# jw007123/hp-Adaptive-Signed-Distance-Field-Octree

Measured on AMD Instinct MI355X. Metric: Query() Mpts/sec at targetError=1e-5 (union3 field, 10M SplitMix64 pts per GPU, HBM-resident); Create() ms reported as create_ms, higher is better.
Workload: dtype f64

## Files before the change

hp-adaptive-signed-distance-field-octree_amd/__init__.py:

```python
import ctypes as C
import os

import numpy as np

_HERE = os.path.dirname(os.path.abspath(__file__))
_WHICH = os.environ.get("HPSDF_LIBRARY", "")
LIB_PATH = os.path.join(_HERE, "lib", "libhpsdf_%s.so" % _WHICH if _WHICH else "libhpsdf.so")
_LIB = None

OK = 0
ERR_INVALID_ARGUMENT = 1
ERR_NO_DEVICE = 2
ERR_HIP = 3
ERR_BAD_BLOCK = 4
ERR_UNSUPPORTED = 5
ERR_STATE = 6
ERR_OUT_OF_MEMORY = 7
ERR_OPEN_MESH = 8
ERR_BUILD_LIMIT = 9
ABI_VERSION = 4
PRIM_SPHERE, PRIM_BOX, PRIM_TORUS_Y, PRIM_PLANE = 0, 1, 2, 3
OP_UNION, OP_INTERSECT, OP_SUBTRACT = 0, 1, 2
JOB_HEADER_DOUBLES = 9
DEFAULT_JOBS_PER_ROUND = 1024
# ... 52 lines not shown
    def as_dict(self):
        return {n: getattr(self, n) for n, _ in self._fields_}


CALLBACK = C.CFUNCTYPE(C.c_double, C.POINTER(C.c_double), C.c_uint64, C.c_void_p)

_SIGNATURES = {
    "hpsdf_config_default": (C.c_int, [C.POINTER(PodConfig)]),
    "hpsdf_last_error": (C.c_char_p, []),
    "hpsdf_version": (C.c_char_p, []),
    "hpsdf_tables_get": (C.c_int, [C.c_void_p] * 7),
    "hpsdf_ctx_create": (C.c_int, [C.c_int, C.c_void_p, C.POINTER(C.c_void_p)]),
    "hpsdf_ctx_destroy": (C.c_int, [C.c_void_p]),
    "hpsdf_ctx_set_stream": (C.c_int, [C.c_void_p, C.c_void_p]),
    "hpsdf_ctx_synchronize": (C.c_int, [C.c_void_p]),
    "hpsdf_ctx_set_fast_fit": (C.c_int, [C.c_void_p, C.c_int]),
    "hpsdf_ctx_set_fit_mode": (C.c_int, [C.c_void_p, C.c_int]),
    "hpsdf_ctx_get_fit_mode": (C.c_int, [C.c_void_p, C.POINTER(C.c_int)]),
    "hpsdf_ctx_set_split_min_degree": (C.c_int, [C.c_void_p, C.c_int]),
    "hpsdf_ctx_set_block_allocator": (None, [C.c_void_p] * 4),
    "hpsdf_field_release_host_copies": (C.c_int, [C.c_void_p]),
    "hpsdf_set_mesh_face_rule": (None, [C.c_int]),
    "hpsdf_get_mesh_face_rule": (C.c_int, []),
    "hpsdf_set_reduction_order": (None, [C.c_int]),
    "hpsdf_get_reduction_order": (C.c_int, []),
    "hpsdf_ctx_stream": (C.c_void_p, [C.c_void_p]),
    "hpsdf_abi_version": (C.c_int, []),
    "hpsdf_ctx_set_reduction_order": (C.c_int, [C.c_void_p, C.c_int]),
    "hpsdf_ctx_get_reduction_order": (C.c_int, [C.c_void_p, C.POINTER(C.c_int)]),
    "hpsdf_ctx_set_mesh_face_rule": (C.c_int, [C.c_void_p, C.c_int]),
    "hpsdf_ctx_get_mesh_face_rule": (C.c_int, [C.c_void_p, C.POINTER(C.c_int)]),
    "hpsdf_ctx_set_build_limits": (C.c_int, [C.c_void_p, C.c_uint64, C.c_uint64]),
    "hpsdf_ctx_get_build_limits": (C.c_int, [C.c_void_p, C.POINTER(C.c_uint64), C.POINTER(C.c_uint64)]),
    "hpsdf_field_create_analytic": (C.c_int, [C.POINTER(Prim), C.c_int, C.POINTER(C.c_void_p)]),
    "hpsdf_field_create_callback": (C.c_int, [CALLBACK, C.c_void_p, C.POINTER(C.c_void_p)]),
    "hpsdf_field_create_mesh": (C.c_int, [C.c_void_p, C.c_void_p, C.c_uint64, C.c_void_p, C.c_uint64,
                                          C.POINTER(C.c_void_p)]),
    "hpsdf_obj_load": (C.c_int, [C.c_char_p, C.POINTER(C.POINTER(C.c_float)), C.POINTER(C.c_uint64),
                                 C.POINTER(C.POINTER(C.c_uint64)), C.POINTER(C.c_uint64)]),
    "hpsdf_field_create_tree_csg": (C.c_int, [C.c_void_p, C.c_int, C.c_void_p, C.POINTER(C.c_void_p)]),
    "hpsdf_field_destroy": (C.c_int, [C.c_void_p]),
    "hpsdf_field_mesh_stats": (C.c_int, [C.c_void_p, C.POINTER(C.c_uint64), C.c_int]),
    "hpsdf_field_mesh_arrays": (C.c_int, [C.c_void_p, C.POINTER(C.c_uint64), C.POINTER(C.c_void_p), C.POINTER(C.c_uint64)]),
    "hpsdf_field_eval_device": (C.c_int, [C.c_void_p, C.c_void_p, C.c_void_p, C.c_size_t, C.c_void_p]),
    "hpsdf_field_eval_host": (C.c_int, [C.c_void_p, C.c_void_p, C.c_void_p, C.c_size_t, C.c_void_p]),
    "hpsdf_field_eval_naive_host": (C.c_int, [C.c_void_p, C.c_void_p, C.c_void_p, C.c_size_t, C.c_void_p]),
    "hpsdf_field_eval_wave_host": (C.c_int, [C.c_void_p, C.c_void_p, C.c_void_p, C.c_size_t, C.c_void_p]),
    "hpsdf_field_eval_lane_host": (C.c_int, [C.c_void_p, C.c_void_p, C.c_void_p, C.c_size_t, C.c_void_p]),
    "hpsdf_selftest_acosf": (C.c_int, [C.c_void_p, C.c_uint32, C.c_uint32, C.c_size_t, C.c_void_p]),
    "hpsdf_selftest_running_total": (C.c_int, [C.c_void_p, C.c_double, C.c_size_t, C.c_int, C.c_int, C.c_void_p, C.c_void_p, C.c_void_p, C.c_void_p]),
    "hpsdf_tree_upload": (C.c_int, [C.c_void_p, C.c_void_p, C.c_size_t, C.POINTER(C.c_void_p)]),
    "hpsdf_tree_destroy": (C.c_int, [C.c_void_p]),
    "hpsdf_tree_info": (C.c_int, [C.c_void_p, C.POINTER(C.c_uint64), C.POINTER(C.c_uint64), C.POINTER(C.c_uint64),
                                  C.POINTER(C.c_int), C.POINTER(C.c_int)]),
    "hpsdf_query_device": (C.c_int, [C.c_void_p, C.c_void_p, C.c_void_p, C.c_size_t, C.c_void_p]),
    "hpsdf_query_host": (C.c_int, [C.c_void_p, C.c_void_p, C.c_void_p, C.c_size_t, C.c_void_p]),
    "hpsdf_query_gradient_device": (C.c_int, [C.c_void_p, C.c_void_p, C.c_void_p, C.c_size_t, C.c_void_p, C.c_void_p]),
    "hpsdf_query_gradient_host": (C.c_int, [C.c_void_p, C.c_void_p, C.c_void_p, C.c_size_t, C.c_void_p, C.c_void_p]),
    "hpsdf_query_true_gradient_device": (C.c_int, [C.c_void_p, C.c_void_p, C.c_void_p, C.c_size_t, C.c_uint32, C.c_void_p, C.c_void_p]),
    "hpsdf_query_true_gradient_host": (C.c_int, [C.c_void_p, C.c_void_p, C.c_void_p, C.c_size_t, C.c_uint32, C.c_void_p, C.c_void_p]),
    "hpsdf_query_true_gradient_block": (C.c_int, [C.c_void_p, C.c_size_t, C.c_void_p, C.c_size_t, C.c_uint32, C.c_void_p, C.c_void_p]),
    "hpsdf_query_hessian_device": (C.c_int, [C.c_void_p, C.c_void_p, C.c_void_p, C.c_size_t, C.c_uint32, C.c_void_p, C.c_void_p, C.c_void_p,
                                             C.c_void_p]),
    "hpsdf_query_hessian_host": (C.c_int, [C.c_void_p, C.c_void_p, C.c_void_p, C.c_size_t, C.c_uint32, C.c_void_p, C.c_void_p, C.c_void_p,
                                           C.c_void_p]),
    "hpsdf_query_hessian_block": (C.c_int, [C.c_void_p, C.c_size_t, C.c_void_p, C.c_size_t, C.c_uint32, C.c_void_p, C.c_void_p, C.c_void_p,
# ... 268 lines not shown
        data = C.string_at(blk, size)
        if obj is None:
            lib()._libc.free(blk)
        return data

    def set_stream(self, stream):
        check(lib().hpsdf_ctx_set_stream(self.handle, C.c_void_p(stream) if stream else None))

    def set_reduction_order(self, left_assoc):
        check(lib().hpsdf_ctx_set_reduction_order(self.handle, -1 if left_assoc is None else (1 if left_assoc else 0)))

    def reduction_order(self):
        v = C.c_int()
        check(lib().hpsdf_ctx_get_reduction_order(self.handle, C.byref(v)))
        return v.value

    def set_mesh_face_rule(self, reference):
        check(lib().hpsdf_ctx_set_mesh_face_rule(self.handle, -1 if reference is None else (1 if reference else 0)))

    def mesh_face_rule(self):
        v = C.c_int()
        check(lib().hpsdf_ctx_get_mesh_face_rule(self.handle, C.byref(v)))
        return v.value

    def set_build_limits(self, max_nodes=0, max_bytes=0):
        none = (1 << 64) - 1
        check(lib().hpsdf_ctx_set_build_limits(self.handle, none if max_nodes is None else int(max_nodes), none if max_bytes is None else int(max_bytes)))

    def build_limits(self):
        a, b = C.c_uint64(), C.c_uint64()
        check(lib().hpsdf_ctx_get_build_limits(self.handle, C.byref(a), C.byref(b)))
        return a.value, b.value

    def set_fast_fit(self, on=True):
        check(lib().hpsdf_ctx_set_fast_fit(self.handle, 1 if on else 0))

    def set_fit_mode(self, mode):
        check(lib().hpsdf_ctx_set_fit_mode(self.handle, int(mode)))

    def set_split_min_degree(self, degree):
        check(lib().hpsdf_ctx_set_split_min_degree(self.handle, int(degree)))

    def fit_mode(self):
        m = C.c_int(0)
        check(lib().hpsdf_ctx_get_fit_mode(self.handle, C.byref(m)))
        return m.value

    def synchronize(self):
        check(lib().hpsdf_ctx_synchronize(self.handle))

    def close(self):
        if self.handle:
            lib().hpsdf_ctx_destroy(self.handle)
            self.handle = C.c_void_p()

    def __del__(self):
        try:
            self.close()
        except Exception:
            pass


BVH_DTYPE = np.dtype([("lo0", np.float32, 3), ("hi0", np.float32, 3), ("lo1", np.float32, 3), ("hi1", np.float32, 3),
                      ("c0", np.int32), ("c1", np.int32), ("pad", np.uint32, 2)])
SLAB_DTYPE = np.dtype([("g0", np.float32, 4), ("n0", np.float32, 4), ("g1", np.float32, 4), ("n1", np.float32, 4)])

# ... 1237 lines not shown
```

hp-adaptive-signed-distance-field-octree_amd/build.py:

```python
import os
import shutil
import subprocess
import sys

HERE = os.path.dirname(os.path.abspath(__file__))
CSRC = os.path.join(HERE, "csrc")
LIBDIR = os.path.join(HERE, "lib")
LIB = os.path.join(LIBDIR, "libhpsdf.so")
HOOKS_LIB = os.path.join(LIBDIR, "libhpsdf_hooks.so")
HOOK_SOURCES = ["frontier_build.cpp", "capi_build.cpp"]
INCLUDE = os.path.normpath(os.path.join(HERE, "..", "include"))

SOURCES = ["fit_mesh.hip", "fit_analytic.hip", "fit_samples.hip", "fit.hip", "kernels.hip", "mesh_field.hip", "frontier.hip", "fit_mfma.hip", "fit_low.hip", "mesh_build.hip", "cg.hip", "continuity_asm.hip", "surface.hip", "surface_sparse.hip", "surface_dual.hip", "query_gradient.hip", "query_hessian.hip", "project.hip", "cast_rays.hip", "query_bounds.hip", "integrate.hip", "integrate_pair.hip", "clearance.hip", "clearance_batch.hip", "simplify.hip", "tables.cpp", "builder.cpp", "mesh.cpp", "obj.cpp", "continuity.cpp", "host_query.cpp", "integrate_pair_host.cpp", "clearance_host.cpp", "simplify_host.cpp", "frontier_build.cpp", "runtime.cpp", "capi_field.cpp", "capi_tree.cpp", "capi_build.cpp", "bench_fit.cpp"]
HEADERS = sorted(f for f in os.listdir(CSRC) if f.endswith(".hpp"))
QUERY_SOURCES = ("kernels.hip",)
MESH_SOURCES = ("mesh_field.hip", "fit_mesh.hip")
SOURCE_GROUPS = {"query": QUERY_SOURCES, "mesh": MESH_SOURCES}
PUBLIC_HEADERS = ["hpsdf.h", "hpsdf_octree.hpp"]

FLAGS = ["-O3", "-std=c++17", "-fPIC", "-ffp-contract=off", "-fno-fast-math", "--offload-arch=gfx950",
         "-fvisibility=hidden", "-Wall", "-Wno-unused-function", "-I", INCLUDE]
FLAGS += os.environ.get("HPSDF_EXTRA_FLAGS", "").split()
FILE_FLAGS = {"fit_mfma.hip": ["-mllvm", "-amdgpu-mfma-vgpr-form=1"]}
for _s in ("query_gradient.hip", "query_hessian.hip", "project.hip", "cast_rays.hip", "surface_dual.hip", "host_query.cpp"):
    FILE_FLAGS[_s] = ["-Wno-pass-failed"]


def hipcc():
    for c in (os.environ.get("HIPCC"), "/opt/rocm/bin/hipcc", shutil.which("hipcc")):
        if c and os.path.exists(c):
            return c
    raise RuntimeError("hipcc not found: the HIP extension cannot be built (there is no CPU fallback)")


def stale():
    if not os.path.exists(LIB) or not os.path.exists(HOOKS_LIB):
        return True
    t = os.path.getmtime(LIB)
    deps = [os.path.join(CSRC, s) for s in SOURCES + HEADERS] + [os.path.join(INCLUDE, h) for h in PUBLIC_HEADERS]
    deps.append(os.path.abspath(__file__))
    return any(os.path.exists(d) and os.path.getmtime(d) > t for d in deps)


def build(force=False, verbose=False):
    if not force and not stale():
        return LIB
# ... 98 lines not shown
```

hp-adaptive-signed-distance-field-octree_amd/csrc/frontier_build.cpp:

```cpp
#include <hip/hip_runtime_api.h>

#include <algorithm>
#include <atomic>
#include <cfloat>
#include <cmath>
#include <cstddef>
#include <chrono>
#include <cstdio>
#include <cstdlib>
#include <cstring>
#include <memory>
#include <string>
#include <vector>

#include "block.hpp"
#include "builder.hpp"
#include "frontier.hpp"
#include "frontier_dev.hpp"
#include "frontier_workspace.hpp"
#include "launch.hpp"
#include "runtime.hpp"

namespace hpsdf {

// ... 4 lines not shown
    asm volatile("yield");
#endif
}

bool frontierEligible(const hpsdf_ctx* ctx, const hpsdf_config* cfg, const hpsdf_field* field, uint64_t K) {
    if (const char* e = std::getenv("HPSDF_HOST_FRONTIER"))
        if (e[0] == '1') return false;
    if (cfg->weighting_type > 2) return false;
    if (cfg->enable_logging) return false;
    const hpsdf_field* in = innermost(field);
    if (!in || (in->kind != kHostAnalytic && in->kind != kHostMesh)) return false;
    if (in->kind == kHostMesh) {
        const char* e = std::getenv("HPSDF_MESH_FUSED");
        if (e && e[0] == '1') return false;
        if (meshFaceRuleReference(ctx)) return false;
    }
    const uint64_t k = K ? K : HPSDF_DEFAULT_JOBS_PER_ROUND;
    return k <= kFrJobs;
}

#define FR_LAUNCH(kernel, launcher, stream, ...)                                            \
    do {                                                                                    \
        const hipError_t le_ = launcher(stream, __VA_ARGS__);                               \
        if (le_ != hipSuccess) return ::hpsdf::hipFail(le_, "launch of " #kernel);          \
        if (frSyncEveryLaunch()) {                                                          \
            std::fprintf(stderr, "[frontier] " #kernel " ...");                             \
            const hipError_t se_ = hipStreamSynchronize(stream);                            \
            std::fprintf(stderr, " %s\n", hipGetErrorString(se_));                          \
        }                                                                                   \
    } while (0)
static bool frSyncEveryLaunch() {
    static const bool on = std::getenv("HPSDF_FRONTIER_SYNC") != nullptr;
    return on;
}

namespace {

inline double frNow() { return std::chrono::duration<double, std::micro>(std::chrono::steady_clock::now().time_since_epoch()).count(); }

inline bool watchWord(const volatile uint32_t* word, uint32_t want, double microseconds) {
    const double limit = frNow() + microseconds;
    while (*word != want && frNow() < limit) frCpuRelax();
    return *word == want;
}

std::vector<size_t> makeLdsTable(bool w) {
    std::vector<size_t> t(kMaxDegree + 1, 0);
    for (int deg = 1; deg <= kMaxDegree; ++deg)
        for (int incr = 0; incr < 2; ++incr) {
            int g, pl;
            frShape(deg, incr != 0, 1u << 20, &g, &pl, false, w);
            for (int gg = 1; gg <= g; ++gg) {
                const int nq = 4 * deg + 1;
                int pp = nq;
                while (pp > 1 && frLds(deg, gg, pp) > kFitChunkLdsBytes) --pp;
                if (w) {
                    const int minPlanes = ((int)frCoef(deg) + 100 + nq * nq - 1) / (nq * nq);
                    pp = std::max(pp, std::min(nq, minPlanes));
                    if (gg > 1 && frLds(deg, gg, pp) > kFitMaxLdsBytes) continue;
                }
                t[deg] = std::max(t[deg], frLds(deg, gg, pp));
            }
        }
    return t;
}
const std::vector<size_t>& fitLdsTable(bool weighted) {
// ... 368 lines not shown
    const volatile uint32_t* roundWord = &hh->round;
    if (!watchWord(roundWord, want, 2.0e3)) {
        HPSDF_HIP(hipStreamSynchronize(s));
        if (*roundWord != want) {
            HPSDF_HIP(hipMemcpy(ws->hostHdr, d.hdr, kFrHdrCopyBytes, hipMemcpyDeviceToHost));
            if (hh->round != want) return fail(HPSDF_ERR_STATE, "frontier: a round ended without advancing");
        }
    }
    std::atomic_thread_fence(std::memory_order_acquire);
    tSync += frNow() - ts;
    return HPSDF_OK;
}

void FrontierBuild::rearmForNextBuild(bool wentOn) {
    ws->clean = frLaunchInit(s, initDev(), T0) == hipSuccess, ws->cleanRank = rank, ws->cleanWorld = world;
    ws->lastWentOn = wentOn;
}

int FrontierBuild::runRound0() {
    int rc;
    hipError_t e = ws->ensureArena(std::max<uint64_t>(1, T0.arenaRows), 0, s);
    if (e == hipSuccess && mesh) e = ws->ensureSamples(std::max<uint64_t>(1, T0.samples), s);
    if (e != hipSuccess) return hipFail(e, "frontier buffers");
    if ((rc = prepareNext(T.nNodes, T0.arenaRows, 2u, 0))) return rc;
    d.target = cfg.target_error_threshold;
    if (!ws->clean || ws->cleanRank != rank || ws->cleanWorld != world) FR_LAUNCH(fr_init_kernel, frLaunchInit, s, initDev(), T0);
    ws->clean = false;
    FieldDev fdr = fd;
    if (mesh) {
        HPSDF_HIP(launchMeshSample(s, r0Tasks, T0.nTasks, 2, ctx->dTables, fd, rm, ws->samples));
        fdr.kind = kFieldSamples;
        fdr.samples = ws->samples;
    }
    HPSDF_HIP(launchFit(s, 2, 1, r0Blocks, T0.nBlocks, r0Lds, r0Tasks, ws->arena, d.errs, world == 1 ? ws->pinnedDev : nullptr, ctx->dTables, fdr, rm));
    if (weighted && (rc = applyWeights(r0Blocks, T0.nBlocks, r0Lds, r0Tasks, nullptr, true, world == 1 ? 0u : (uint32_t)rank * stride0,
                                       T0.sliceFirst[rank + 1] - T0.sliceFirst[rank])))
        return rc;
    if (replica) {
        if (pending.rowsBytes != (size_t)part0 * sizeof(double)) return fail(HPSDF_ERR_STATE, "frontier: round 0's part of the arena");
        pending.rowsEntered();
        if ((rc = exchange(ws->arena, pending.rowsBytes, "round 0's rows"))) return rc;
    }
    if ((rc = exchange(d.errs, (size_t)stride0 * sizeof(double), "round 0"))) return rc;
    pending.afterRound0Exchanges(strideK);
    d.errStride = strideK;
    return HPSDF_OK;
}

int FrontierBuild::closeRoundAndOpenNext() {
    int rc;
    pre = (uint64_t)knownNodes + 8ull * Kj <= inlineNodes;
    splitCur = splitOpen, tooLargeCur = samplesTooLarge;
    FrDev dk = d;
    dk.splitFit = splitFitCur = splitCur ? std::max(2, ctx->splitMinDegree) : 0;
    if (rounds == 0) {
        dk.batchIdx = ws->tmplLeaves, dk.batchErr = ws->tmplErr, dk.jobP = r0JobP, dk.jobH = r0JobP;
        dk.errStride = stride0;
    }
    FR_LAUNCH(fr_round_kernel, frLaunchRound, s, dk, rounds == 0 ? T.nLeaves : Kj, (pre ? 1 : 0) | (ws->lastWentOn && pre ? 2 : 0));
    const bool noBlind = std::getenv("HPSDF_FRONTIER_NO_BLIND") != nullptr;
    blind = (rounds >= 1 || ws->lastWentOn) && pre && world == 1 && !weighted && !frSyncEveryLaunch() && !noBlind;
    if (blind) {
        if (mesh && tooLargeCur) return fail(HPSDF_ERR_UNSUPPORTED, "round too large for the sampled mesh path");
        d.splitFit = splitFitCur;
        FrDev de = d;
        FR_LAUNCH(fr_emit_kernel, frLaunchEmit, s, de, Kj);
        if ((rc = launchRoundFits(std::min<uint32_t>(knownMaxDeg + 1u, kMaxDegree), splitCur))) return rc;
// ... 206 lines not shown
```

hp-adaptive-signed-distance-field-octree_amd/csrc/launch.hpp:

```cpp
#pragma once
#include <algorithm>
#include <vector>
#include <hip/hip_runtime_api.h>

#include <cstddef>
#include <cstdint>
#include <cstdlib>
#include <type_traits>

#include "device_types.hpp"

namespace hpsdf {

constexpr unsigned kQueryMaxGrid = 256 * 8 * 4;
constexpr size_t kQueryFewPoints = 256;
inline unsigned gridFor(size_t n) {
    size_t blocks = (n + 255) / 256;
    static const size_t capEnv = [] { const char* e = std::getenv("HPSDF_QUERY_GRID"); return e ? (size_t)std::max(1, std::atoi(e)) : (size_t)0; }();
    const size_t cap = capEnv ? capEnv : kQueryMaxGrid;
    return (unsigned)(blocks < 1 ? 1 : (blocks > cap ? cap : blocks));
}
template <int P, int... Rest, class F>
inline void forMaxDegree(int maxDegree, F&& f) {
    if constexpr (sizeof...(Rest) > 0)
// ... 38 lines not shown
struct IntegrateArgs;
int integrateOnDevice(hpsdf_ctx* ctx, const ClsTree& t, int maxDegree, const IntegrateCell* dLeaves, uint32_t nLeaves, const IntegrateArgs& a,
                      hpsdf_integral* out, hpsdf_integrate_cell** outCells, uint64_t* outCount);
struct PairArgs;
int integratePairOnDevice(hpsdf_ctx* ctx, const ClsTree& tA, const ClsTree& tB, int maxDegree, const IntegrateCell* dLeaves, uint32_t nLeaves,
                          const PairArgs& p, const IntegrateArgs& a, hpsdf_integral* out, hpsdf_integrate_cell** outCells, uint64_t* outCount);
struct ClearanceArgs;
int clearanceOnDevice(hpsdf_ctx* ctx, const ClsTree& tA, const ClsTree& tB, int maxDegree, const IntegrateCell* dLeaves, uint32_t nLeaves,
                      const PairArgs& p, const ClearanceArgs& a, hpsdf_clearance* out, hpsdf_integrate_cell** outCells, uint64_t* outCount);
int clearanceBatchOnDevice(hpsdf_ctx* ctx, const ClsTree& tA, const ClsTree& tB, int maxDegree, const IntegrateCell* dLeaves, uint32_t nLeaves,
                           const double* poses, size_t n, double isoA, uint32_t maxLeaves, const ClearanceArgs& a, uint32_t maxTotalCells,
                           hpsdf_clearance* out);
constexpr size_t kFitMaxLdsBytes = 60 * 1024;
constexpr int kFitBlockThreads = 256;
constexpr int kFitThreads = 256;
constexpr size_t kFitChunkLdsBytes = 40 * 1024;
size_t fitLdsBytes(int degree, int nTasks, int planes);
struct FitShape {
    int cells;
    int cellsPerThread;
    int planes;
    size_t ldsBytes;
};
FitShape fitShape(int degree, int nrows, uint32_t count, bool weighted, bool latencyBound = false);
hipError_t launchFit(hipStream_t stream, int degree, int cellsPerThread, const FitBlock* dBlocks, uint32_t nBlocks, size_t ldsBytes,
                     const FitTask* dTasks, double* dArena, double* dErrs, double* dMirror,
                     const DeviceTables* dTables, const FieldDev& field, const RootMap& rm, const uint32_t* dRange = nullptr);
hipError_t launchFitMulti(hipStream_t stream, const FitBlock* dBlocks, uint32_t maxBlocks, size_t ldsBytes, const FitTask* dTasks,
                          double* dArena, double* dErrs, const DeviceTables* dTables, const FieldDev& field, const RootMap& rm,
                          const uint32_t* dCount);
hipError_t launchFieldEval(hipStream_t stream, const FieldDev& f, const DeviceTables* dTables, const double* dXyz,
                           size_t n, double* dOut);
hipError_t launchPack(hipStream_t stream, const PackItem* dItems, uint32_t nItems, const double* dArena, double* dOut);
hipError_t launchMeshSample(hipStream_t stream, const FitTask* dTasks, uint32_t nTasks, int degree, const DeviceTables* dTables,
                            const FieldDev& field, const RootMap& rm, double* dSamples);
hipError_t launchMeshSampleRange(hipStream_t stream, const FitTask* dTasks, const uint32_t* dRange, uint32_t maxTasks, int degree,
                                 const DeviceTables* dTables, const FieldDev& field, const RootMap& rm, double* dSamples);
constexpr int kMfmaCells = 16;
bool fitMfmaSupports(int degree, const FieldDev& field);
hipError_t launchFitMfma(hipStream_t stream, int degree, const FitBlock* dBlocks, uint32_t nBlocks, const FitTask* dTasks, double* dArena,
                         double* dErrs, const DeviceTables* dTables, const FieldDev& field, const RootMap& rm, const uint32_t* dRange = nullptr);
int fitSplitDefaultMinDegree();
bool fitSplitSupports(int degree, int minDegree);
hipError_t launchFitLow(hipStream_t stream, int degree, const FitTask* dTasks, const uint32_t* dRange, uint32_t first, uint32_t count,
                        uint32_t maxTasks, double* dArena, const DeviceTables* dTables, const double* dSamples);
hipError_t launchFitMfmaLow(hipStream_t stream, int degree, const FitTask* dTasks, const uint32_t* dRange, uint32_t first, uint32_t count,
                            uint32_t maxTasks, double* dArena, const DeviceTables* dTables, const double* dSamples, const RootMap& rm, int leftAssoc);
hipError_t launchMeshEvalWave(hipStream_t stream, const FieldDev& f, const double* dXyz, size_t n, double* dOut);
void meshEvalHostPoints(const MeshDev& hm, const double* xyz, size_t n, double* out);
hipError_t launchMeshNaive(hipStream_t stream, const FieldDev& f, const double* dXyz, size_t n, double* dOut, unsigned long long* dKeys = nullptr);
hipError_t launchAcosfSelftest(hipStream_t stream, uint32_t first, uint32_t stride, size_t n, float* dOut);
constexpr int kTriRecordFloats = 12;
constexpr int kTriPreFloats = 12;
hipError_t launchMeshTriPos(hipStream_t stream, const float* dVerts, const uint32_t* dTris, uint64_t nTris, float* dTriPos,
                            const uint32_t* dSlotTri, float* dTriPre);
hipError_t sortPairsU32(hipStream_t stream, void* tmp, size_t& tmpBytes, const uint32_t* keys, uint32_t* keysOut, const uint32_t* vals, uint32_t* valsOut,
                        size_t n, unsigned bits);
hipMemPool_t meshPool(int dev);
void meshPoolTrim(int dev);
constexpr uint64_t kCgChunk = 256;
inline double cgChunkSum(const double* e, uint64_t count) {
    double v[64];
    for (uint64_t l = 0; l < 64; ++l) {
        auto at = [&](uint64_t i) { return i < count ? e[i] : 0.0; };
        v[l] = ((at(l) + at(64 + l)) + at(128 + l)) + at(192 + l);
    }
// ... 42 lines not shown
```

hp-adaptive-signed-distance-field-octree_amd/csrc/runtime.cpp:

```cpp
#include <hip/hip_runtime_api.h>

#include <algorithm>
#include <cmath>
#include <cstdio>
#include <cstring>
#include <limits>
#include <thread>

#include "launch.hpp"
#include "runtime.hpp"

using namespace hpsdf;

namespace hpsdf {

static thread_local std::string g_lastError;

void setError(const std::string& msg) { g_lastError = msg; }
int fail(int code, const std::string& msg) {
    g_lastError = msg;
    return code;
}
int hipFail(hipError_t e, const char* what) {
    g_lastError = std::string(what) + ": " + hipGetErrorString(e);
// ... 224 lines not shown
        hipEvent_t done = nullptr;
        HPSDF_HIP(hipEventCreateWithFlags(&done, hipEventDisableTiming));
        hipError_t e = hipEventRecord(done, c->stream);
        if (e == hipSuccess) e = hipStreamWaitEvent(next, done, 0);
        (void)hipEventDestroy(done);
        if (e != hipSuccess) return hipFail(e, "hpsdf_ctx_set_stream: ordering the new stream behind the old one");
    }
    c->stream = next;
    return HPSDF_OK;
}

int hpsdf_ctx_set_fit_mode(hpsdf_ctx* c, int mode) {
    if (!c) return fail(HPSDF_ERR_INVALID_ARGUMENT, "null context");
    if (mode != HPSDF_FIT_EXACT && mode != HPSDF_FIT_SPLIT && mode != HPSDF_FIT_FAST) return fail(HPSDF_ERR_INVALID_ARGUMENT, "unknown fit mode");
    c->fitMode = mode;
    return HPSDF_OK;
}
int hpsdf_ctx_get_fit_mode(hpsdf_ctx* c, int* mode) {
    if (!c || !mode) return fail(HPSDF_ERR_INVALID_ARGUMENT, "null argument");
    *mode = c->fitMode;
    return HPSDF_OK;
}
int hpsdf_ctx_set_build_limits(hpsdf_ctx* c, uint64_t max_nodes, uint64_t max_bytes) {
    if (!c) return fail(HPSDF_ERR_INVALID_ARGUMENT, "null context");
    c->limitNodes = max_nodes, c->limitBytes = max_bytes;
    return HPSDF_OK;
}
int hpsdf_ctx_get_build_limits(const hpsdf_ctx* c, uint64_t* max_nodes, uint64_t* max_bytes) {
    if (!c) return fail(HPSDF_ERR_INVALID_ARGUMENT, "null context");
    if (max_nodes) *max_nodes = c->limitNodes;
    if (max_bytes) *max_bytes = c->limitBytes;
    return HPSDF_OK;
}
int hpsdf_ctx_set_split_min_degree(hpsdf_ctx* c, int degree) {
    if (!c) return fail(HPSDF_ERR_INVALID_ARGUMENT, "null context");
    if (degree < 2 || degree > 12) return fail(HPSDF_ERR_INVALID_ARGUMENT, "split_min_degree: 2..12 (12 = never split)");
    c->splitMinDegree = degree;
    return HPSDF_OK;
}
void hpsdf_set_mesh_face_rule(int reference) { setMeshFaceRuleReference(reference); }
int hpsdf_get_mesh_face_rule(void) { return meshFaceRuleReference(nullptr); }
void hpsdf_set_reduction_order(int left_assoc) { setReductionLeftAssoc(left_assoc); }
int hpsdf_get_reduction_order(void) { return reductionLeftAssoc(nullptr); }
int hpsdf_ctx_set_reduction_order(hpsdf_ctx* c, int left_assoc) {
    if (!c) return fail(HPSDF_ERR_INVALID_ARGUMENT, "null context");
    if (left_assoc < -1 || left_assoc > 1) return fail(HPSDF_ERR_INVALID_ARGUMENT, "reduction order: -1 (the process-wide setting), 0 or 1");
    c->reductionOrder = left_assoc;
    return HPSDF_OK;
}
int hpsdf_ctx_get_reduction_order(const hpsdf_ctx* c, int* left_assoc) {
    if (!c || !left_assoc) return fail(HPSDF_ERR_INVALID_ARGUMENT, "null argument");
    *left_assoc = reductionLeftAssoc(c);
    return HPSDF_OK;
}
int hpsdf_ctx_set_mesh_face_rule(hpsdf_ctx* c, int reference) {
    if (!c) return fail(HPSDF_ERR_INVALID_ARGUMENT, "null context");
    if (reference < -1 || reference > 1) return fail(HPSDF_ERR_INVALID_ARGUMENT, "mesh face rule: -1 (the process-wide setting), 0 or 1");
    c->meshFaceRule = reference;
    return HPSDF_OK;
}
int hpsdf_ctx_get_mesh_face_rule(const hpsdf_ctx* c, int* reference) {
    if (!c || !reference) return fail(HPSDF_ERR_INVALID_ARGUMENT, "null argument");
    *reference = meshFaceRuleReference(c);
    return HPSDF_OK;
}
int hpsdf_ctx_set_fast_fit(hpsdf_ctx* c, int on) { return hpsdf_ctx_set_fit_mode(c, on ? HPSDF_FIT_FAST : HPSDF_FIT_EXACT); }
// ... 17 lines not shown
```

hp-adaptive-signed-distance-field-octree_amd/csrc/runtime.hpp:

```cpp
#pragma once
#include <cstdlib>
#include <hip/hip_runtime_api.h>

#include <cstdint>
#include <atomic>
#include <exception>
#include <memory>
#include <mutex>
#include <new>
#include <string>
#include <vector>

#include "device_types.hpp"
#include "tables.hpp"

namespace hpsdf {

template <typename T>
struct Staged {
    T* dev = nullptr;
    T* host = nullptr;
    uint64_t cap = 0;
    hipError_t ensure(uint64_t n) {
        if (n <= cap) return hipSuccess;
// ... 42 lines not shown
    void release() {
        if (device >= 0) (void)hipSetDevice(device);
        if (arena) (void)hipFree(arena);
        arena = nullptr;
        arenaCap = 0;
        tasks.release();
        blocks.release();
        errs.release();
        samples.release();
        if (meshSamples) (void)hipFree(meshSamples);
        meshSamples = nullptr;
        meshSamplesCap = 0;
        pack.release();
        items.release();
    }
};

}

namespace hpsdf {
struct IntegrateCell;
}

struct hpsdf_ctx {
    int device = 0;
    hipStream_t stream = nullptr;
    bool ownsStream = false;
    hpsdf::DeviceTables* dTables = nullptr;
    int fitMode = HPSDF_FIT_SPLIT;
    int splitMinDegree = 6;
    int reductionOrder = -1;
    int meshFaceRule = -1;
    uint64_t limitNodes = 0, limitBytes = 0;
    hpsdf::Workspace ws;
    std::shared_ptr<void> frontierScratch;
    std::shared_ptr<void> continuityScratch;
    char* hostDev = nullptr;
    size_t hostDevCap = 0;
    char* hostPin = nullptr;
    char* hostPinDev = nullptr;
    size_t hostPinCap = 0;
    std::mutex hostLock;
    std::mutex scratchLock;
    uint32_t* dDefer = nullptr;
    uint64_t deferCap = 0;
    uint32_t* dDeferCount = nullptr;
    void* (*blockAlloc)(size_t, void*) = nullptr;
    void (*blockRelease)(void*, void*) = nullptr;
    void* blockUser = nullptr;
    void* allocBlock(size_t bytes) const { return blockAlloc ? blockAlloc(bytes, blockUser) : std::malloc(bytes); }
    void freeBlock(void* p) const {
        if (p == nullptr) return;
        if (blockAlloc) {
            if (blockRelease) blockRelease(p, blockUser);
        } else {
            std::free(p);
        }
    }
};

struct hpsdf_tree {
    int device = 0;
    hpsdf::NodeRec* dNodes = nullptr;
    hpsdf::TopEntry* dTop = nullptr;
    hpsdf::NodeRec* dTopRec = nullptr;
    double* dCoeffs = nullptr;
// ... 142 lines not shown
```

include/hpsdf.h:

```cpp
#ifndef HPSDF_H
#define HPSDF_H

#include <stddef.h>
#include <stdint.h>

#ifdef __cplusplus
extern "C" {
#endif

#if defined(__GNUC__)
#define HPSDF_API __attribute__((visibility("default")))
#else
#define HPSDF_API
#endif

typedef enum hpsdf_status {
    HPSDF_OK = 0,
    HPSDF_ERR_INVALID_ARGUMENT = 1,
    HPSDF_ERR_NO_DEVICE = 2,
    HPSDF_ERR_HIP = 3,
    HPSDF_ERR_BAD_BLOCK = 4,
    HPSDF_ERR_UNSUPPORTED = 5,
    HPSDF_ERR_STATE = 6,
    HPSDF_ERR_OUT_OF_MEMORY = 7,
// ... 31 lines not shown
    double continuity_strength;
    uint8_t enable_logging;
    uint8_t pad2[7];
    double target_error_threshold;
    uint64_t thread_count;
    float root_min[3];
    float root_max[3];
} hpsdf_config;

HPSDF_API int hpsdf_config_default(hpsdf_config* out);

HPSDF_API const char* hpsdf_last_error(void);
HPSDF_API const char* hpsdf_version(void);

HPSDF_API int hpsdf_tables_get(double* roots, double* weights, double* normalised_lengths, double* recurrence,
                               uint64_t* coeff_count, uint64_t* basis_index, uint64_t* sum_to_n);

typedef struct hpsdf_ctx hpsdf_ctx;
HPSDF_API int hpsdf_ctx_create(int device, void* stream, hpsdf_ctx** out);
HPSDF_API int hpsdf_ctx_destroy(hpsdf_ctx* ctx);
HPSDF_API int hpsdf_ctx_set_stream(hpsdf_ctx* ctx, void* stream);
HPSDF_API int hpsdf_ctx_synchronize(hpsdf_ctx* ctx);
enum { HPSDF_FIT_EXACT = 0, HPSDF_FIT_SPLIT = 1, HPSDF_FIT_FAST = 2 };
HPSDF_API int hpsdf_ctx_set_fit_mode(hpsdf_ctx* ctx, int mode);
HPSDF_API int hpsdf_ctx_get_fit_mode(hpsdf_ctx* ctx, int* mode);
HPSDF_API int hpsdf_ctx_set_split_min_degree(hpsdf_ctx* ctx, int degree);
HPSDF_API int hpsdf_ctx_set_fast_fit(hpsdf_ctx* ctx, int on);
HPSDF_API void hpsdf_set_reduction_order(int left_assoc);
HPSDF_API int hpsdf_get_reduction_order(void);
HPSDF_API int hpsdf_ctx_set_reduction_order(hpsdf_ctx* ctx, int left_assoc);
HPSDF_API int hpsdf_ctx_get_reduction_order(const hpsdf_ctx* ctx, int* left_assoc);
HPSDF_API int hpsdf_ctx_set_build_limits(hpsdf_ctx* ctx, uint64_t max_nodes, uint64_t max_bytes);
HPSDF_API int hpsdf_ctx_get_build_limits(const hpsdf_ctx* ctx, uint64_t* max_nodes, uint64_t* max_bytes);
HPSDF_API void* hpsdf_ctx_stream(hpsdf_ctx* ctx);

enum { HPSDF_PRIM_SPHERE = 0, HPSDF_PRIM_BOX = 1, HPSDF_PRIM_TORUS_Y = 2, HPSDF_PRIM_PLANE = 3 };
enum { HPSDF_OP_UNION = 0, HPSDF_OP_INTERSECT = 1, HPSDF_OP_SUBTRACT = 2 };
#define HPSDF_MAX_PRIMS 16
typedef struct hpsdf_prim {
    int32_t kind;
    int32_t op;
    double p[8];
} hpsdf_prim;

typedef double (*hpsdf_callback)(const double* pt, uint64_t thread_idx, void* user);

typedef struct hpsdf_field hpsdf_field;
typedef struct hpsdf_tree hpsdf_tree;

HPSDF_API int hpsdf_field_create_analytic(const hpsdf_prim* prims, int n_prims, hpsdf_field** out);
HPSDF_API int hpsdf_field_create_callback(hpsdf_callback cb, void* user, hpsdf_field** out);
HPSDF_API int hpsdf_field_create_mesh(hpsdf_ctx* ctx, const float* verts, uint64_t n_verts, const uint64_t* tris,
                                      uint64_t n_tris, hpsdf_field** out);
HPSDF_API int hpsdf_obj_load(const char* path, float** verts, uint64_t* n_verts, uint64_t** tris, uint64_t* n_tris);
HPSDF_API int hpsdf_field_create_tree_csg(const hpsdf_tree* old_tree, int op, const hpsdf_field* inner,
                                          hpsdf_field** out);
HPSDF_API int hpsdf_field_destroy(hpsdf_field* f);
HPSDF_API int hpsdf_field_eval_device(hpsdf_ctx* ctx, const hpsdf_field* f, const double* d_xyz, size_t n,
                                      double* d_out);
HPSDF_API int hpsdf_field_eval_host(hpsdf_ctx* ctx, const hpsdf_field* f, const double* xyz, size_t n, double* out);
HPSDF_API int hpsdf_field_release_host_copies(hpsdf_field* f);
HPSDF_API void hpsdf_set_mesh_face_rule(int reference);
HPSDF_API int hpsdf_get_mesh_face_rule(void);
HPSDF_API int hpsdf_ctx_set_mesh_face_rule(hpsdf_ctx* ctx, int reference);
HPSDF_API int hpsdf_ctx_get_mesh_face_rule(const hpsdf_ctx* ctx, int* reference);
HPSDF_API int hpsdf_field_eval_naive_host(hpsdf_ctx* ctx, const hpsdf_field* f, const double* xyz, size_t n, double* out);
// ... 308 lines not shown
```

Baseline: 94030.

## Add packed multi-cell coarse fit kernel for the degree-2 first round

New measurement: 94200 (median of 5 runs). No clear change (+0.2%).

```diff
diff --git a/hp-adaptive-signed-distance-field-octree_amd/__init__.py b/hp-adaptive-signed-distance-field-octree_amd/__init__.py
--- a/hp-adaptive-signed-distance-field-octree_amd/__init__.py
+++ b/hp-adaptive-signed-distance-field-octree_amd/__init__.py
@@ -108,6 +108,7 @@
     "hpsdf_ctx_get_mesh_face_rule": (C.c_int, [C.c_void_p, C.POINTER(C.c_int)]),
     "hpsdf_ctx_set_build_limits": (C.c_int, [C.c_void_p, C.c_uint64, C.c_uint64]),
     "hpsdf_ctx_get_build_limits": (C.c_int, [C.c_void_p, C.POINTER(C.c_uint64), C.POINTER(C.c_uint64)]),
+    "hpsdf_ctx_coarse_fit_launches": (C.c_uint64, [C.c_void_p]),
     "hpsdf_field_create_analytic": (C.c_int, [C.POINTER(Prim), C.c_int, C.POINTER(C.c_void_p)]),
     "hpsdf_field_create_callback": (C.c_int, [CALLBACK, C.c_void_p, C.POINTER(C.c_void_p)]),
     "hpsdf_field_create_mesh": (C.c_int, [C.c_void_p, C.c_void_p, C.c_uint64, C.c_void_p, C.c_uint64,
@@ -442,6 +443,9 @@
         check(lib().hpsdf_ctx_get_build_limits(self.handle, C.byref(a), C.byref(b)))
         return a.value, b.value
 
+    def coarse_fit_launches(self):
+        return int(lib().hpsdf_ctx_coarse_fit_launches(self.handle))
+
     def set_fast_fit(self, on=True):
         check(lib().hpsdf_ctx_set_fast_fit(self.handle, 1 if on else 0))
 
diff --git a/hp-adaptive-signed-distance-field-octree_amd/build.py b/hp-adaptive-signed-distance-field-octree_amd/build.py
--- a/hp-adaptive-signed-distance-field-octree_amd/build.py
+++ b/hp-adaptive-signed-distance-field-octree_amd/build.py
@@ -11,7 +11,7 @@
 HOOK_SOURCES = ["frontier_build.cpp", "capi_build.cpp"]
 INCLUDE = os.path.normpath(os.path.join(HERE, "..", "include"))
 
-SOURCES = ["fit_mesh.hip", "fit_analytic.hip", "fit_samples.hip", "fit.hip", "kernels.hip", "mesh_field.hip", "frontier.hip", "fit_mfma.hip", "fit_low.hip", "mesh_build.hip", "cg.hip", "continuity_asm.hip", "surface.hip", "surface_sparse.hip", "surface_dual.hip", "query_gradient.hip", "query_hessian.hip", "project.hip", "cast_rays.hip", "query_bounds.hip", "integrate.hip", "integrate_pair.hip", "clearance.hip", "clearance_batch.hip", "simplify.hip", "tables.cpp", "builder.cpp", "mesh.cpp", "obj.cpp", "continuity.cpp", "host_query.cpp", "integrate_pair_host.cpp", "clearance_host.cpp", "simplify_host.cpp", "frontier_build.cpp", "runtime.cpp", "capi_field.cpp", "capi_tree.cpp", "capi_build.cpp", "bench_fit.cpp"]
+SOURCES = ["fit_mesh.hip", "fit_analytic.hip", "fit_samples.hip", "coarse_fit.hip", "fit.hip", "kernels.hip", "mesh_field.hip", "frontier.hip", "fit_mfma.hip", "fit_low.hip", "mesh_build.hip", "cg.hip", "continuity_asm.hip", "surface.hip", "surface_sparse.hip", "surface_dual.hip", "query_gradient.hip", "query_hessian.hip", "project.hip", "cast_rays.hip", "query_bounds.hip", "integrate.hip", "integrate_pair.hip", "clearance.hip", "clearance_batch.hip", "simplify.hip", "tables.cpp", "builder.cpp", "mesh.cpp", "obj.cpp", "continuity.cpp", "host_query.cpp", "integrate_pair_host.cpp", "clearance_host.cpp", "simplify_host.cpp", "frontier_build.cpp", "runtime.cpp", "capi_field.cpp", "capi_tree.cpp", "capi_build.cpp", "bench_fit.cpp"]
 HEADERS = sorted(f for f in os.listdir(CSRC) if f.endswith(".hpp"))
 QUERY_SOURCES = ("kernels.hip",)
 MESH_SOURCES = ("mesh_field.hip", "fit_mesh.hip")
diff --git a/hp-adaptive-signed-distance-field-octree_amd/csrc/coarse_fit.hip b/hp-adaptive-signed-distance-field-octree_amd/csrc/coarse_fit.hip
--- /dev/null
+++ b/hp-adaptive-signed-distance-field-octree_amd/csrc/coarse_fit.hip
@@ -0,0 +1,167 @@
+#include <hip/hip_runtime.h>
+
+#include <algorithm>
+#include <cstdint>
+
+#include "device_types.hpp"
+#include "field_glue.hpp"
+#include "launch.hpp"
+
+namespace hpsdf {
+
+constexpr int kCoarseCells = 16;
+constexpr int kCoarseThreads = 64 * kCoarseCells;
+constexpr int kCoarseNq = 9, kCoarseNq2 = 81, kCoarseSamples = 729, kCoarseRows = 10;
+constexpr int kCoarseUnitPlanes = 3;
+constexpr int kCoarseUnitsPerCell = kCoarseNq2 * (kCoarseNq / kCoarseUnitPlanes);
+static_assert(kCoarseCells <= 16, "the sums' lane map packs 16 lanes a row");
+static_assert(kCoarseNq % kCoarseUnitPlanes == 0, "whole units");
+static_assert(16 * kCoarseRows <= kCoarseThreads, "a lane per (cell, row)");
+
+constexpr size_t coarseFitLdsBytes() {
+    return (size_t)kCoarseCells * kCoarseSamples * sizeof(double);
+}
+
+template <int KIND, bool LEFT>
+__global__ __launch_bounds__(kCoarseThreads) void coarse_fit_kernel(const FitTask* __restrict__ tasks, uint32_t nTasks, uint32_t cells,
+                                                                    double* __restrict__ arena, double* __restrict__ errs,
+                                                                    double* __restrict__ mirror, const DeviceTables* __restrict__ T,
+                                                                    FieldDev field, RootMap rm) {
+    extern __shared__ double lds[];
+    __shared__ double sNl[13 * 11];
+    __shared__ double sRec[26];
+    __shared__ double sT[3 * kCoarseNq];
+    __shared__ double sR[kCoarseNq], sW[kCoarseNq];
+    __shared__ double sC[kCoarseCells * 8];
+    __shared__ double sOut[kCoarseCells * kCoarseRows];
+    __shared__ unsigned char sB[kCoarseRows][4];
+    double* sF = lds;
+
+    constexpr int nq = kCoarseNq, nq2 = kCoarseNq2;
+    constexpr int gl = nq * (nq - 1) / 2;
+    const int tid = threadIdx.x;
+    const uint32_t firstTask = blockIdx.x * cells;
+    const int G = (int)min(cells, nTasks - firstTask);
+    const int depth = tasks[firstTask].depth;
+
+    stageQueryTables(T, sNl, sRec);
+    if (tid < nq) {
+        const int q = tid;
+        const double x = T->roots[gl + q];
+        sR[q] = x;
+        sW[q] = T->weights[gl + q];
+        double m2 = 0.0, m1 = 1.0;
+        sT[q] = 1.0;
+        for (int i = 1; i <= 2; ++i) {
+            const double l = T->rec[i][0] * x * m1 - T->rec[i][1] * m2;
+            m2 = m1, m1 = l;
+            sT[i * nq + q] = l;
+        }
+    }
+    if (tid >= 64 && tid < 64 + G) {
+        const int g = tid - 64;
+        const FitTask& tk = tasks[firstTask + g];
+        double sc[3];
+        for (int a = 0; a < 3; ++a) {
+            sc[a] = (double)(tk.bmax[a] - tk.bmin[a]) * 0.5;
+            sC[8 * g + 3 + a] = (double)((tk.bmin[a] + tk.bmax[a]) / 2.0f);
+            sC[8 * g + a] = sc[a];
+        }
+        sC[8 * g + 6] = prod3<LEFT>(sc[0], sc[1], sc[2]);
+        sC[8 * g + 7] = __longlong_as_double((long long)tk.sampleOff);
+    }
+    if (tid >= 128 && tid < 128 + kCoarseRows * 4) (&sB[0][0])[tid - 128] = (&T->bidx[0][0])[tid - 128];
+    __syncthreads();
+
+    {
+        constexpr int thirds = nq / kCoarseUnitPlanes;
+        const int units = G * kCoarseUnitsPerCell;
+        uint32_t meshHint = 0xFFFFFFFFu;
+        for (int u = tid; u < units; u += kCoarseThreads) {
+            const int g = u / kCoarseUnitsPerCell, rem = u - g * kCoarseUnitsPerCell;
+            const int jk = rem / thirds, i0 = (rem - jk * thirds) * kCoarseUnitPlanes, j = jk / nq, k = jk - j * nq;
+            const double* c = sC + 8 * g;
+            const double uy = sR[j] * c[1] + c[4], uz = sR[k] * c[2] + c[5];
+            const double wy = uy * rm.bounds[1] + rm.centre[1];
+            const double wz = uz * rm.bounds[2] + rm.centre[2];
+            const double wj = sW[j], wk = sW[k], c6 = c[6];
+            const uint64_t sbase = (uint64_t)__double_as_longlong(c[7]) + (uint64_t)(j * nq + k);
+            for (int il = 0; il < kCoarseUnitPlanes; ++il) {
+                const int i = i0 + il;
+                const double ux = sR[i] * c[0] + c[3];
+                const double wx = ux * rm.bounds[0] + rm.centre[0];
+                const uint64_t sidx = sbase + (uint64_t)(i * nq2);
+                const double fv = fieldEvalWorld<KIND, false, LEFT>(field, wx, wy, wz, sidx, sNl, sRec, meshHint);
+                sF[g * kCoarseSamples + i * nq2 + jk] = c6 * prod3<LEFT>(sW[i], wj, wk) * fv;
+            }
+        }
+    }
+    __syncthreads();
+
+    const int cell = tid & 15, row = tid >> 4;
+    const bool act = row < kCoarseRows && cell < G;
+    if (act) {
+        const double* F = sF + cell * kCoarseSamples;
+        double acc = 0.0;
+        const int i0 = sB[row][0], i1 = sB[row][1], i2 = sB[row][2];
+        const double n0 = sNl[i0 * 11 + depth], n1 = sNl[i1 * 11 + depth], n2 = sNl[i2 * 11 + depth];
+        double tk[nq];
+#pragma unroll
+        for (int k = 0; k < nq; ++k) tk[k] = sT[i2 * nq + k];
+        for (int i = 0; i < nq; ++i) {
+            const double a0 = sT[i0 * nq + i] * n0;
+            for (int j = 0; j < nq; ++j) {
+                const double a1 = a0 * sT[i1 * nq + j] * n1;
+                const double* Fr = F + i * nq2 + j * nq;
+                double lp[nq], f[nq];
+#pragma unroll
+                for (int k = 0; k < nq; ++k) lp[k] = a1 * tk[k] * n2, f[k] = Fr[k];
+#pragma unroll
+                for (int k = 0; k < nq; ++k) acc = acc + lp[k] * f[k];
+            }
+        }
+        const uint64_t at = tasks[firstTask + cell].outOff + (uint64_t)row;
+        arena[at] = acc;
+        if (mirror != nullptr) mirror[at] = acc;
+        sOut[cell * kCoarseRows + row] = acc;
+    }
+    __syncthreads();
+    if (tid < G) {
+        double e = 0.0;
+        for (int r = (int)T->count[1]; r < kCoarseRows; ++r)
+            if (sB[r][3] == 2) {
+                const double c = sOut[tid * kCoarseRows + r];
+                e = e + c * c;
+            }
+        errs[tasks[firstTask + tid].errSlot] = e;
+    }
+}
+
+template <int KIND, bool LEFT>
+static hipError_t launchCoarseFitT(hipStream_t stream, const FitTask* dTasks, uint32_t nTasks, uint32_t cells, double* dArena, double* dErrs,
+                                   double* dMirror, const DeviceTables* dTables, const FieldDev& field, const RootMap& rm) {
+    constexpr size_t lds = coarseFitLdsBytes();
+    const hipError_t ae = hipFuncSetAttribute((const void*)coarse_fit_kernel<KIND, LEFT>, hipFuncAttributeMaxDynamicSharedMemorySize, (int)lds);
+    if (ae != hipSuccess) return ae;
+    hipLaunchKernelGGL((coarse_fit_kernel<KIND, LEFT>), dim3((nTasks + cells - 1) / cells), dim3(kCoarseThreads), lds, stream, dTasks, nTasks, cells,
+                       dArena, dErrs, dMirror, dTables, field, rm);
+    return hipGetLastError();
+}
+
+bool coarseFitSupports(const FieldDev& field) {
+    return field.csgOp < 0 && (field.kind == kFieldAnalytic || field.kind == kFieldSamples);
+}
+
+hipError_t launchCoarseFit(hipStream_t stream, const FitTask* dTasks, uint32_t nTasks, double* dArena, double* dErrs, double* dMirror,
+                           const DeviceTables* dTables, const FieldDev& field, const RootMap& rm) {
+    if (nTasks == 0) return hipSuccess;
+    if (!coarseFitSupports(field)) return hipErrorInvalidValue;
+    const uint32_t cells = std::min<uint32_t>((uint32_t)kCoarseCells, std::max<uint32_t>(1u, (nTasks + 255u) / 256u));
+#define HPSDF_COARSE_LAUNCH(K)                                                                                                         \
+    (field.leftAssoc ? launchCoarseFitT<K, true>(stream, dTasks, nTasks, cells, dArena, dErrs, dMirror, dTables, field, rm)              \
+                     : launchCoarseFitT<K, false>(stream, dTasks, nTasks, cells, dArena, dErrs, dMirror, dTables, field, rm))
+    return field.kind == kFieldAnalytic ? HPSDF_COARSE_LAUNCH(kFieldAnalytic) : HPSDF_COARSE_LAUNCH(kFieldSamples);
+#undef HPSDF_COARSE_LAUNCH
+}
+
+}
diff --git a/hp-adaptive-signed-distance-field-octree_amd/csrc/frontier_build.cpp b/hp-adaptive-signed-distance-field-octree_amd/csrc/frontier_build.cpp
--- a/hp-adaptive-signed-distance-field-octree_amd/csrc/frontier_build.cpp
+++ b/hp-adaptive-signed-distance-field-octree_amd/csrc/frontier_build.cpp
@@ -60,6 +60,10 @@
 static bool frSyncEveryLaunch() {
     static const bool on = std::getenv("HPSDF_FRONTIER_SYNC") != nullptr;
     return on;
+}
+static bool frCoarseFit() {
+    const char* e = std::getenv("HPSDF_COARSE_FIT");
+    return !(e && e[0] == '0');
 }
 
 namespace {
@@ -494,7 +498,13 @@
         fdr.kind = kFieldSamples;
         fdr.samples = ws->samples;
     }
-    HPSDF_HIP(launchFit(s, 2, 1, r0Blocks, T0.nBlocks, r0Lds, r0Tasks, ws->arena, d.errs, world == 1 ? ws->pinnedDev : nullptr, ctx->dTables, fdr, rm));
+    double* const mirror = world == 1 ? ws->pinnedDev : nullptr;
+    if (!weighted && frCoarseFit() && coarseFitSupports(fdr)) {
+        HPSDF_HIP(launchCoarseFit(s, r0Tasks, T0.nTasks, ws->arena, d.errs, mirror, ctx->dTables, fdr, rm));
+        ++ctx->coarseFitLaunches;
+    } else {
+        HPSDF_HIP(launchFit(s, 2, 1, r0Blocks, T0.nBlocks, r0Lds, r0Tasks, ws->arena, d.errs, mirror, ctx->dTables, fdr, rm));
+    }
     if (weighted && (rc = applyWeights(r0Blocks, T0.nBlocks, r0Lds, r0Tasks, nullptr, true, world == 1 ? 0u : (uint32_t)rank * stride0,
                                        T0.sliceFirst[rank + 1] - T0.sliceFirst[rank])))
         return rc;
diff --git a/hp-adaptive-signed-distance-field-octree_amd/csrc/launch.hpp b/hp-adaptive-signed-distance-field-octree_amd/csrc/launch.hpp
--- a/hp-adaptive-signed-distance-field-octree_amd/csrc/launch.hpp
+++ b/hp-adaptive-signed-distance-field-octree_amd/csrc/launch.hpp
@@ -94,6 +94,9 @@
 hipError_t launchFieldEval(hipStream_t stream, const FieldDev& f, const DeviceTables* dTables, const double* dXyz,
                            size_t n, double* dOut);
 hipError_t launchPack(hipStream_t stream, const PackItem* dItems, uint32_t nItems, const double* dArena, double* dOut);
+bool coarseFitSupports(const FieldDev& field);
+hipError_t launchCoarseFit(hipStream_t stream, const FitTask* dTasks, uint32_t nTasks, double* dArena, double* dErrs, double* dMirror,
+                           const DeviceTables* dTables, const FieldDev& field, const RootMap& rm);
 hipError_t launchMeshSample(hipStream_t stream, const FitTask* dTasks, uint32_t nTasks, int degree, const DeviceTables* dTables,
                             const FieldDev& field, const RootMap& rm, double* dSamples);
 hipError_t launchMeshSampleRange(hipStream_t stream, const FitTask* dTasks, const uint32_t* dRange, uint32_t maxTasks, int degree,
diff --git a/hp-adaptive-signed-distance-field-octree_amd/csrc/runtime.cpp b/hp-adaptive-signed-distance-field-octree_amd/csrc/runtime.cpp
--- a/hp-adaptive-signed-distance-field-octree_amd/csrc/runtime.cpp
+++ b/hp-adaptive-signed-distance-field-octree_amd/csrc/runtime.cpp
@@ -280,6 +280,7 @@
     if (max_bytes) *max_bytes = c->limitBytes;
     return HPSDF_OK;
 }
+uint64_t hpsdf_ctx_coarse_fit_launches(const hpsdf_ctx* c) { return c ? c->coarseFitLaunches : 0; }
 int hpsdf_ctx_set_split_min_degree(hpsdf_ctx* c, int degree) {
     if (!c) return fail(HPSDF_ERR_INVALID_ARGUMENT, "null context");
     if (degree < 2 || degree > 12) return fail(HPSDF_ERR_INVALID_ARGUMENT, "split_min_degree: 2..12 (12 = never split)");
diff --git a/hp-adaptive-signed-distance-field-octree_amd/csrc/runtime.hpp b/hp-adaptive-signed-distance-field-octree_amd/csrc/runtime.hpp
--- a/hp-adaptive-signed-distance-field-octree_amd/csrc/runtime.hpp
+++ b/hp-adaptive-signed-distance-field-octree_amd/csrc/runtime.hpp
@@ -98,6 +98,7 @@
     int reductionOrder = -1;
     int meshFaceRule = -1;
     uint64_t limitNodes = 0, limitBytes = 0;
+    uint64_t coarseFitLaunches = 0;
     hpsdf::Workspace ws;
     std::shared_ptr<void> frontierScratch;
     std::shared_ptr<void> continuityScratch;
diff --git a/include/hpsdf.h b/include/hpsdf.h
--- a/include/hpsdf.h
+++ b/include/hpsdf.h
@@ -87,6 +87,7 @@
 HPSDF_API int hpsdf_ctx_get_reduction_order(const hpsdf_ctx* ctx, int* left_assoc);
 HPSDF_API int hpsdf_ctx_set_build_limits(hpsdf_ctx* ctx, uint64_t max_nodes, uint64_t max_bytes);
 HPSDF_API int hpsdf_ctx_get_build_limits(const hpsdf_ctx* ctx, uint64_t* max_nodes, uint64_t* max_bytes);
+HPSDF_API uint64_t hpsdf_ctx_coarse_fit_launches(const hpsdf_ctx* ctx);
 HPSDF_API void* hpsdf_ctx_stream(hpsdf_ctx* ctx);
 
 enum { HPSDF_PRIM_SPHERE = 0, HPSDF_PRIM_BOX = 1, HPSDF_PRIM_TORUS_Y = 2, HPSDF_PRIM_PLANE = 3 };
```
